# maxrmorrison/torbi

Hardware: AMD Instinct MI355X
Metric: timesteps decoded/sec, 1440 states batch=512 (higher is better)
Workload: dtype f32; 1 GPU; 1440 states, 500 frames, batch=512 per GPU, fp32, dense transition (BASELINE configs[2]); decode = forward + argmax + backtrace, inputs resident in HBM; parallelism=single GPU, streams=2

## Files before the change

torbi_amd/csrc/resident_forward.hpp:

```cpp
#pragma once

#include <hip/hip_runtime.h>
#include <stdint.h>
#include <math.h>
#include <type_traits>

#include "pruned_forward.hpp"
#include "lazy_backtrace.hpp"
#include "nonfinite.hpp"

namespace resident {

using pruned::kBlk;
using pruned::kR;
using pruned::kTop;
using pruned::ListBlock;
using pruned::group_bcast;
using pruned::load_list_block;

constexpr int kNI = 16;
constexpr int kMaxBatches = 16;
constexpr int kRowGroup = 16;
#ifndef TORBI_TILE16_MAX_S
#define TORBI_TILE16_MAX_S pruned::kMaxS16
// ... 100 lines not shown
    if (b >= jb.B) return;
    int f = jb.frames[b];
    f = f < 1 ? 1 : (f > jb.T ? jb.T : f);
    atomicAdd(&jb.hist[f], 1);
}

__global__ __launch_bounds__(1024) void order_large_scan_kernel(OrderJob jb, int ascending) {
    __shared__ int part[1024];
    const int T = jb.T, tid = threadIdx.x;
    const int per = (T + 1024) / 1024;
    auto length_at = [&](int k) { return ascending ? 1 + k : T - k; };
    int sum = 0;
    for (int k = tid * per; k < (tid + 1) * per && k < T; ++k) sum += jb.hist[length_at(k)];
    part[tid] = sum;
    __syncthreads();
    if (tid == 0) {
        int run = 0;
        for (int i = 0; i < 1024; ++i) { const int v = part[i]; part[i] = run; run += v; }
    }
    __syncthreads();
    int run = part[tid];
    for (int k = tid * per; k < (tid + 1) * per && k < T; ++k) {
        const int f = length_at(k), v = jb.hist[f];
        jb.hist[f] = run;
        run += v;
    }
}

__global__ __launch_bounds__(256) void order_large_place_kernel(OrderJob jb) {
    const int b = blockIdx.x * 256 + threadIdx.x;
    if (b >= jb.B) return;
    int f = jb.frames[b];
    f = f < 1 ? 1 : (f > jb.T ? jb.T : f);
    jb.order[atomicAdd(&jb.hist[f], 1)] = b;
}

__global__ __launch_bounds__(256) void order_tiles_kernel(OrderJobs jobs) {
    __shared__ __align__(16) int s_len[kOrderChunk];
    const int w = blockIdx.x * 256 + threadIdx.x;
    if (w < 128) jobs.stats[w] = 0u;
    for (int k = w; k < jobs.nflags; k += gridDim.x * 256) jobs.flags[k] = 0u;
    if ((int)blockIdx.x * 256 >= jobs.tiles) return;
    auto batch_of_tile = [&](int v) {
        int k = 0;
        for (int q = 1; q < jobs.n; ++q)
            if (v >= jobs.job[q].tile0) k = q;
        return k;
    };
    auto tile_length = [&](int k, int j) {
        const OrderJob &jb = jobs.job[k];
        const int last = jobs.ni * j + jobs.ni - 1 < jb.B ? jobs.ni * j + jobs.ni - 1 : jb.B - 1;
        int f = jb.frames[jb.order[jobs.ascending ? last : jobs.ni * j]];
        return f < 1 ? 1 : (f > jb.T ? jb.T : f);
    };
    const bool live = w < jobs.tiles;
    const int k = live ? batch_of_tile(w) : 0;
    const int j = w - jobs.job[k].tile0;
    const int mine = live ? tile_length(k, j) : 1;
    int rank = 0;
    for (int v0 = 0; v0 < jobs.tiles; v0 += kOrderChunk) {
        const int n = min(kOrderChunk, jobs.tiles - v0), n4 = (n + 3) / 4 * 4;
        if (v0) __syncthreads();
        for (int v = threadIdx.x; v < n4; v += 256) {
            const int kv = v < n ? batch_of_tile(v0 + v) : 0;
            s_len[v] = v < n ? tile_length(kv, v0 + v - jobs.job[kv].tile0) : 0;
        }
        __syncthreads();
        for (int v = 0; v < n4; v += 4) {
            const int4 g = *reinterpret_cast<const int4 *>(&s_len[v]);
            rank += (g.x > mine) || (g.x == mine && v0 + v < w);
            rank += (g.y > mine) || (g.y == mine && v0 + v + 1 < w);
            rank += (g.z > mine) || (g.z == mine && v0 + v + 2 < w);
            rank += (g.w > mine) || (g.w == mine && v0 + v + 3 < w);
        }
    }
    if (live) jobs.tile_map[jobs.ascending ? jobs.tiles - 1 - rank : rank] = (k << 20) | j;
}

__global__ __launch_bounds__(256) void absent_kernel(uint4 *__restrict__ slots, size_t granules) {
    const uint4 a = {kAbsentBits, kAbsentBits, kAbsentBits, kAbsentBits};
    for (size_t g = (size_t)blockIdx.x * 256 + threadIdx.x; g < granules; g += (size_t)gridDim.x * 256) slots[g] = a;
}

__device__ __forceinline__ u64 top_key(float v, int state) {
    unsigned u = __float_as_uint(v);
    u ^= (u >> 31) ? 0xffffffffu : 0x80000000u;
    return ((u64)u << 32) | (unsigned)(0x7fffffff - state);
}

template <int KTOP = kTop>
__device__ __forceinline__ void top_insert(u64 *list, u64 x) {
    if (x <= list[KTOP - 1]) return;
#pragma unroll
    for (int r = 0; r < KTOP; ++r) {
        if (x != 0ull) {
            const u64 old = atomicMax(&list[r], x);
            x = old < x ? old : (old == x ? 0ull : x);
        }
    }
}

typedef unsigned int v4u __attribute__((ext_vector_type(4)));
__device__ __forceinline__ void store_through(__amdgpu_buffer_rsrc_t buffer, int offset, float4 v) {
    v4u x = {__float_as_uint(v.x), __float_as_uint(v.y), __float_as_uint(v.z), __float_as_uint(v.w)};
    __builtin_amdgcn_raw_buffer_store_b128(x, buffer, offset, 0, 16);
}
__device__ __forceinline__ void store_plain(__amdgpu_buffer_rsrc_t buffer, int offset, float4 v) {
    v4u x = {__float_as_uint(v.x), __float_as_uint(v.y), __float_as_uint(v.z), __float_as_uint(v.w)};
    __builtin_amdgcn_raw_buffer_store_b128(x, buffer, offset, 0, 0);
}
__device__ __forceinline__ float4 load_through(__amdgpu_buffer_rsrc_t buffer, int offset) {
    const v4u x = __builtin_amdgcn_raw_buffer_load_b128(buffer, offset, 0, 16);
    return make_float4(__uint_as_float(x.x), __uint_as_float(x.y), __uint_as_float(x.z), __uint_as_float(x.w));
}
__device__ __forceinline__ __amdgpu_buffer_rsrc_t buffer_of(const void *base, unsigned bytes) {
    return __builtin_amdgcn_make_buffer_rsrc(const_cast<void *>(base), 0, (int)bytes, 0x00020000);
}

#ifndef RESIDENT_ABL
#define RESIDENT_ABL 0
#endif
#ifndef CLUSTER_POLL_SLEEP
#define CLUSTER_POLL_SLEEP 4
#endif
#ifndef CLUSTER_ROUND
#define CLUSTER_ROUND 8
#endif
#ifndef RESIDENT_EXTRA_VALU
#define RESIDENT_EXTRA_VALU 0
#endif
#ifndef RESIDENT_HORIZON
#define RESIDENT_HORIZON 1
#endif
#ifndef RESIDENT_HORIZON_SLACK
#define RESIDENT_HORIZON_SLACK 2
#endif

#ifndef RESIDENT_PRIO
#define RESIDENT_PRIO 1
#endif
#ifndef RESIDENT_PRIO_CAP
#define RESIDENT_PRIO_CAP 3
#endif
__device__ __forceinline__ int prio_level(int left) {
    const int level = left >= 6 ? 3 : left >= 4 ? 2 : left >= 2 ? 1 : 0;
    return level < RESIDENT_PRIO_CAP ? level : RESIDENT_PRIO_CAP;
}
#ifndef RESIDENT_DEPTH
#define RESIDENT_DEPTH 1
#endif
#ifndef RESIDENT_SPLIT_ADDS
#define RESIDENT_SPLIT_ADDS 0
#endif
constexpr int scan_depth(int MAXP, int KR, bool CLUSTER, int NI) {
    const bool fits = KR == 1 ? !(MAXP == 11 && NI == 8) && !(MAXP == 6 && CLUSTER) : MAXP == 1;
    return RESIDENT_DEPTH >= 2 && fits ? 2 : 1;
}

#ifdef RESIDENT_STAMP
constexpr int kPhases = 12;
__device__ unsigned long long g_phase[1024 * 16 * kPhases];
__device__ unsigned long long g_wgtime[1024 * 4];
#define RSTAMP(i) { const unsigned long long now_ = __builtin_readcyclecounter(); acc[i] += now_ - last; last = now_; }
#define RCOUNT(i, n) acc[i] += (n)
#else
#define RSTAMP(i)
#define RCOUNT(i, n)
#endif

template <int KW, int MAXP, bool PIPE, int KR = kR, bool CLUSTER = false, int NI = 16, bool REPAIR = false>
__global__ __launch_bounds__(64 * KW) void resident_forward_kernel(Group grp, Cluster clu, const float *__restrict__ tt,
                                                                   const float2 *__restrict__ sorted,
                                                                   const float *__restrict__ initial, int S, int SpP) {
    constexpr int kNI = NI, G = NI / 4, EPL = kBlk / G, kRowGroup = 64 / G;
    constexpr int kR = KR, kTop = KR + 1;
    static_assert(NI == 16 || NI == 8, "tiles of 16 or 8 items");
    extern __shared__ __attribute__((aligned(16))) float lds[];
    const int S4 = (S + 3) / 4 * 4;
    u64 *top = reinterpret_cast<u64 *>(lds + (size_t)kNI * S4);
    float *mtopv = reinterpret_cast<float *>(top + kNI * kTop);
    int *mtopi = reinterpret_cast<int *>(mtopv + kNI * kTop);
    int *sframes = mtopi + kNI * kTop;
    int *sitem = sframes + kNI;
    int *smisc = sitem + kNI;

    const int tid = threadIdx.x, lane = tid & 63;
    const int wave = __builtin_amdgcn_readfirstlane(tid >> 6);
    const unsigned long long clock_0 = clock64(), wall_0 = wall_clock64();
#ifdef RESIDENT_STAMP
    const unsigned long long wg_start = wall_clock64();
#endif

    int cid = blockIdx.x, member = 0;
    const int R = CLUSTER ? clu.R : 1;
    if constexpr (REPAIR) {
        if (!grp.only || grp.only[blockIdx.x] == 0u) return;
    }
    bool local = false;
    if constexpr (CLUSTER) {
        const int cls = blockIdx.x & 7;
        if (tid == 0) {
            smisc[0] = (int)__hip_atomic_fetch_add(clu.control + cls, 1u, __ATOMIC_RELAXED, __HIP_MEMORY_SCOPE_AGENT);
            smisc[1] = 0;
        }
        __syncthreads();
        const int ticket = __builtin_amdgcn_readfirstlane(smisc[0]);
        if (clu.spread) {
            const int per = R / 8;
            member = cls * per + ticket % per;
            cid = ticket / per;
        } else {
            member = ticket % R;
            cid = (ticket / R) * 8 + cls;
        }
        if (cid >= clu.tiles) return;
        if (wave == 0) {
            unsigned *const where = clu.where + (size_t)cid * kMaxR;
            const unsigned xcc = __builtin_amdgcn_s_getreg(20 | (0 << 6) | (3 << 11)) & 15u;
            if (lane == 0) __hip_atomic_store(where + member, xcc + 1u, __ATOMIC_RELAXED, __HIP_MEMORY_SCOPE_AGENT);
            unsigned long long since = 0ull;
            unsigned seen = xcc + 1u;
            bool complete = true;
            for (;;) {
                if (lane < R) seen = __hip_atomic_load(where + lane, __ATOMIC_RELAXED, __HIP_MEMORY_SCOPE_AGENT);
                if (__all(seen != 0u)) break;
                const unsigned long long now = wall_clock64();
                if (since == 0ull) since = now;
                if (now - since >= clu.wait_ticks) { complete = false; break; }
                __builtin_amdgcn_s_sleep(8);
            }
            const bool same = complete && __all(seen == xcc + 1u);
            if (lane == 0) smisc[2] = same ? 1 : 0;
        }
        __syncthreads();
#ifndef CLUSTER_LOCAL_EXCHANGE
#define CLUSTER_LOCAL_EXCHANGE 1
#endif
        local = CLUSTER_LOCAL_EXCHANGE && smisc[2] != 0;
    }
    const int code = grp.tile_map[cid];
    const Batch &bat = grp.batch[code >> 20];
    const float *__restrict__ obs = bat.obs;
    float *__restrict__ hist = bat.hist;
    const int B = bat.B, T = bat.T;
    const int b0 = (code & 0xfffff) * kNI;
    bool odd = false;

    if (tid < kNI) {
        int f = 0;
        const int item = bat.order[b0 + tid < B ? b0 + tid : B - 1];
        if (b0 + tid < B) {
            f = bat.frames[item];
            f = f < 1 ? 1 : (f > T ? T : f);
        }
        sframes[tid] = f;
        sitem[tid] = item;
    }
    if (tid < kNI * kTop) top[tid] = 0ull;
    __syncthreads();
    int fmax = 0;
#pragma unroll
    for (int it = 0; it < kNI; ++it) fmax = max(fmax, sframes[it]);

    for (int item = 0; item < kNI; ++item) {
        const int b = sitem[item];
        const bool valid = b0 + item < B;
        const float *src = obs + (size_t)b * T * S;
        float *dst = hist + (size_t)b * T * S;
        for (int i = tid; i < S; i += 64 * KW) {
            const float v = src[i] + initial[i];
            odd = odd || nonfinite::odd(v);
            lds[i * kNI + item] = v;
            if (valid) dst[i] = v;
            top_insert<kTop>(top + item * kTop, top_key(v, i));
        }
    }

    const int g = lane & (G - 1);
    const int jl = G == 4 ? (int)((0xFBAE9DC873261540ull >> (4 * (lane >> 2))) & 15)
                          : (int)((0xFE7654DC32BA9810ull >> (4 * ((lane >> 1) & 15))) & 15) + (lane & 32) / 2;
    const char *ptile = reinterpret_cast<const char *>(lds) + 16 * g;
    const int nrg = (S + kRowGroup - 1) / kRowGroup;
    const int rg_lo = CLUSTER ? cluster_first_group(member, nrg, R) : 0;
    const int rg_hi = CLUSTER ? cluster_first_group(member + 1, nrg, R) : nrg;
    const unsigned xrow = (unsigned)S4 * kNI * (unsigned)sizeof(float);
    const unsigned xbytes = (unsigned)cluster_slot_bytes(S);
    static_assert(kTop <= kMaxTop, "a member publishes at most kMaxTop list entries per item");
    int ib[4];
#pragma unroll
    for (int it = 0; it < 4; ++it) ib[it] = sitem[4 * g + it];

    float pend[MAXP][4];
    const int own_lo = kRowGroup * rg_lo, own_hi = kRowGroup * rg_hi < S ? kRowGroup * rg_hi : S;
    const int pieces = CLUSTER ? (S - (own_hi - own_lo)) * G : 0;
    auto place = [&](int c) {
        int row = c / G;
        row = row < own_lo ? row : row + (own_hi - own_lo);
        return (row * kNI + 4 * (c % G)) * 4;
    };
#ifndef RESIDENT_FIXED8
#define RESIDENT_FIXED8 1
#endif
#ifndef RESIDENT_FIXED16
#define RESIDENT_FIXED16 1
#endif
    constexpr bool FIXED = CLUSTER && MAXP == 1 && (NI == 16 ? RESIDENT_FIXED16 : RESIDENT_FIXED8);
    ListBlock<EPL> head0, head1;
    float obnext[4] = {0.f, 0.f, 0.f, 0.f};
    if constexpr (FIXED) {
        const int rg = rg_lo + wave;
        const int jj = kRowGroup * rg + jl;
        const int jr = (rg < rg_hi && jj < S) ? jj : S - 1;
        const float2 *row = sorted + (size_t)jr * SpP + EPL * g;
        load_list_block(head0, row, 0);
        load_list_block(head1, row, kBlk);
        if (fmax > 1) {
#pragma unroll
            for (int it = 0; it < 4; ++it) obnext[it] = obs[((size_t)ib[it] * T + 1) * S + jr];
        }
    }
    unsigned stat_blocks = 0, stat_passes = 0;
    int horizon[MAXP];
#pragma unroll
    for (int p = 0; p < MAXP; ++p) horizon[p] = 1;

    auto publish_top = [&](int row) {
        if (tid < kNI * kTop) {
            const u64 key = top[tid];
            unsigned u = (unsigned)(key >> 32);
            u ^= (u >> 31) ? 0x80000000u : 0xffffffffu;
            const float value = key ? __uint_as_float(u) : -INFINITY;
            mtopv[tid] = value;
            mtopi[tid] = key ? (0x7fffffff - (int)(unsigned)key) * S : 0;
            top[tid] = 0ull;
            const int item = tid / kTop;
            if (tid == item * kTop && member == 0 && b0 + item < B && row < sframes[item])
                bat.rowmax[(size_t)sitem[item] * T + row] = value;
        }
    };
    __syncthreads();
    publish_top(0);
#ifdef RESIDENT_STAMP
    unsigned long long acc[kPhases] = {};
    unsigned long long last = __builtin_readcyclecounter();
#endif

    constexpr int kPrio = (CLUSTER || REPAIR || MAXP > 8) ? 0 : RESIDENT_PRIO;
    const int npass = __builtin_amdgcn_readfirstlane(wave < nrg ? (nrg - wave + KW - 1) / KW : 0);
    if constexpr (kPrio == 2) {
        if (npass > nrg / KW) __builtin_amdgcn_s_setprio(1);
    }

    for (int t = 1; t < fmax; ++t) {
        __syncthreads();
        RSTAMP(0);

        float seedv[4][kR ? kR : 1], thr[4];
        int seedo[4][kR ? kR : 1];
        bool live[4];
#pragma unroll
        for (int it = 0; it < 4; ++it) {
            const int item = 4 * g + it;
            live[it] = t < sframes[item];
            if constexpr (kTop == 4) {
                const float4 v = *reinterpret_cast<const float4 *>(mtopv + item * kTop);
                const int4 o = *reinterpret_cast<const int4 *>(mtopi + item * kTop);
                const float vv[4] = {v.x, v.y, v.z, v.w};
                const int oo[4] = {o.x, o.y, o.z, o.w};
#pragma unroll
                for (int r = 0; r < kR; ++r) { seedv[it][r] = vv[r]; seedo[it][r] = oo[r]; }
                thr[it] = live[it] ? vv[kR] : -INFINITY;
            } else {
#pragma unroll
                for (int r = 0; r < kR; ++r) { seedv[it][r] = mtopv[item * kTop + r]; seedo[it][r] = mtopi[item * kTop + r]; }
                thr[it] = live[it] ? mtopv[item * kTop + kR] : -INFINITY;
            }
        }
        RSTAMP(1);

        int opaque = 0;
        asm volatile("" : "+s"(opaque));
#pragma unroll
        for (int p = 0; p < MAXP; ++p) {
            const int rg = rg_lo + wave + KW * p + opaque;
            if (rg < rg_hi) {
                if constexpr (kPrio == 1) {
                    const int left = npass - p;
                    const int level = prio_level(left);
                    if (p == 0 || level != prio_level(left + 1)) {
                        if (level == 3) __builtin_amdgcn_s_setprio(3);
                        else if (level == 2) __builtin_amdgcn_s_setprio(2);
                        else if (level == 1) __builtin_amdgcn_s_setprio(1);
                        else if (p != 0) __builtin_amdgcn_s_setprio(0);
                    }
                }
                const int jj = kRowGroup * rg + jl;
                const bool jv = jj < S;
                const int jr = jv ? jj : S - 1;
                const float2 *row = sorted + (size_t)jr * SpP + EPL * g;
                ListBlock<EPL> cur, nxt;
                float ob[4];
                if constexpr (FIXED) {
                    cur = head0;
                    nxt = head1;
#pragma unroll
                    for (int it = 0; it < 4; ++it) ob[it] = obnext[it];
                } else {
                    load_list_block(cur, row, 0);
                    load_list_block(nxt, row, kBlk);
#pragma unroll
                    for (int it = 0; it < 4; ++it)
                        ob[it] = (RESIDENT_ABL & 32) ? 0.5f * it : obs[((size_t)ib[it] * T + t) * S + jr];
                }
                float seedt[4][kR ? kR : 1];
#pragma unroll
                for (int it = 0; it < 4; ++it)
#pragma unroll
                    for (int r = 0; r < kR; ++r)
                        seedt[it][r] = (RESIDENT_ABL & 64) ? -1.0f : tt[(unsigned)(seedo[it][r] + jr)];

                float best[4] = {-INFINITY, -INFINITY, -INFINITY, -INFINITY};
#if RESIDENT_EXTRA_VALU
                float dummy[4] = {0.f, 0.f, 0.f, 0.f};
#endif
                struct PairData { float4 p0, p1; float t0, t1; };
                auto issue = [&](auto Hc, const ListBlock<EPL> &blk, PairData &d) {
                    constexpr int H = decltype(Hc)::value, O = H / (EPL / 2), E = H % (EPL / 2);
                    float t0, t1;
                    int o0, o1;
                    if (RESIDENT_ABL & 4) {
                        t0 = blk.e[E].x; t1 = blk.e[E].z; o0 = __float_as_int(blk.e[E].y); o1 = __float_as_int(blk.e[E].w);
                    } else {
                        t0 = group_bcast<G, O>(blk.e[E].x); t1 = group_bcast<G, O>(blk.e[E].z);
                        o0 = group_bcast<G, O>(__float_as_int(blk.e[E].y));
                        o1 = group_bcast<G, O>(__float_as_int(blk.e[E].w));
                    }
                    asm volatile("" : "+v"(t0), "+v"(t1));
                    d.t0 = t0; d.t1 = t1;
                    if (RESIDENT_ABL & 2) {
                        d.p0 = make_float4(__int_as_float(o0), t1, t0, t1);
                        d.p1 = make_float4(__int_as_float(o1), t0, t1, t0);
                    } else {
                        d.p0 = *reinterpret_cast<const float4 *>(ptile + o0);
                        d.p1 = *reinterpret_cast<const float4 *>(ptile + o1);
                    }
                };
                auto math = [&](const PairData &d) {
#if RESIDENT_EXTRA_VALU
#pragma unroll
                    for (int x = 0; x < RESIDENT_EXTRA_VALU; ++x) asm volatile("v_add_f32 %0, %0, %1" : "+v"(dummy[x & 3]) : "v"(d.t0));
#endif
                    if (RESIDENT_SPLIT_ADDS) {
                        float a0 = d.t0 + d.p0.x, a1 = d.t0 + d.p0.y, a2 = d.t0 + d.p0.z, a3 = d.t0 + d.p0.w;
                        float b0 = d.t1 + d.p1.x, b1 = d.t1 + d.p1.y, b2 = d.t1 + d.p1.z, b3 = d.t1 + d.p1.w;
                        asm volatile("" : "+v"(a0), "+v"(a1), "+v"(a2), "+v"(a3), "+v"(b0), "+v"(b1), "+v"(b2), "+v"(b3));
                        best[0] = fmaxf(fmaxf(best[0], a0), b0);
                        best[1] = fmaxf(fmaxf(best[1], a1), b1);
                        best[2] = fmaxf(fmaxf(best[2], a2), b2);
                        best[3] = fmaxf(fmaxf(best[3], a3), b3);
                        return;
                    }
                    best[0] = fmaxf(fmaxf(best[0], d.t0 + d.p0.x), d.t1 + d.p1.x);
                    best[1] = fmaxf(fmaxf(best[1], d.t0 + d.p0.y), d.t1 + d.p1.y);
                    best[2] = fmaxf(fmaxf(best[2], d.t0 + d.p0.z), d.t1 + d.p1.z);
                    best[3] = fmaxf(fmaxf(best[3], d.t0 + d.p0.w), d.t1 + d.p1.w);
                };
                PairData ahead;
                PairData ahead1;
                constexpr int kDepth = PIPE ? scan_depth(MAXP, KR, CLUSTER, NI) : 1;
                auto consume = [&](const ListBlock<EPL> &blk, const ListBlock<EPL> &after) {
                    if constexpr (kDepth == 2) {
                        PairData fresh;
#define TORBI_STAGE(H_, BLK_)                                                                  \
                        issue(std::integral_constant<int, (H_ + 2) % 8>(), BLK_, fresh);       \
                        __builtin_amdgcn_sched_barrier(0);                                     \
                        math(ahead);                                                           \
                        __builtin_amdgcn_sched_barrier(0);                                     \
                        ahead = ahead1;                                                        \
                        ahead1 = fresh;
                        TORBI_STAGE(0, blk)
                        TORBI_STAGE(1, blk)
                        TORBI_STAGE(2, blk)
                        TORBI_STAGE(3, blk)
                        TORBI_STAGE(4, blk)
                        TORBI_STAGE(5, blk)
                        TORBI_STAGE(6, after)
                        TORBI_STAGE(7, after)
#undef TORBI_STAGE
                    } else if (PIPE) {
                        PairData other;
#define TORBI_STAGE(H_, CUR_, NXT_)                                                   \
                        issue(std::integral_constant<int, H_ + 1>(), blk, NXT_);      \
                        __builtin_amdgcn_sched_barrier(0);                            \
                        math(CUR_);                                                   \
                        __builtin_amdgcn_sched_barrier(0);
                        TORBI_STAGE(0, ahead, other)
                        TORBI_STAGE(1, other, ahead)
                        TORBI_STAGE(2, ahead, other)
                        TORBI_STAGE(3, other, ahead)
                        TORBI_STAGE(4, ahead, other)
                        TORBI_STAGE(5, other, ahead)
                        TORBI_STAGE(6, ahead, other)
#undef TORBI_STAGE
                        issue(std::integral_constant<int, 0>(), after, ahead);
                        __builtin_amdgcn_sched_barrier(0);
                        math(other);
                        __builtin_amdgcn_sched_barrier(0);
                    } else {
                        PairData d;
                        issue(std::integral_constant<int, 0>(), blk, d); math(d);
                        issue(std::integral_constant<int, 1>(), blk, d); math(d);
                        issue(std::integral_constant<int, 2>(), blk, d); math(d);
                        issue(std::integral_constant<int, 3>(), blk, d); math(d);
                        issue(std::integral_constant<int, 4>(), blk, d); math(d);
                        issue(std::integral_constant<int, 5>(), blk, d); math(d);
                        issue(std::integral_constant<int, 6>(), blk, d); math(d);
                        issue(std::integral_constant<int, 7>(), blk, d); math(d);
                    }
                };
                if (PIPE) issue(std::integral_constant<int, 0>(), cur, ahead);
                if constexpr (kDepth == 2) issue(std::integral_constant<int, 1>(), cur, ahead1);
                int nblk = 1;
                consume(cur, nxt);
                load_list_block(cur, row, 2 * kBlk);
                auto fold_seeds = [&]() {
#pragma unroll
                    for (int it = 0; it < 4; ++it)
#pragma unroll
                        for (int r = 0; r < kR; ++r) best[it] = fmaxf(best[it], seedv[it][r] + seedt[it][r]);
                };
                const int first_test = RESIDENT_HORIZON ? horizon[p] : 1;
                auto more = [&](const ListBlock<EPL> &blk) {
                    if (RESIDENT_ABL & 1) return nblk < 11;
                    if (RESIDENT_HORIZON && nblk < first_test) return true;
                    const float tn = group_bcast<G, 0>(blk.e[0].x);
                    return (bool)__any(jv && ((tn + thr[0] > best[0]) | (tn + thr[1] > best[1]) | (tn + thr[2] > best[2]) |
                                              (tn + thr[3] > best[3])));
                };
                const int Sp = (S + 15) / 16 * 16;
                fold_seeds();
                RSTAMP(2);
                for (int kk = kBlk; kk < Sp; kk += 2 * kBlk) {
                    if (!more(nxt)) break;
                    RCOUNT(7, 1);
                    ++nblk;
                    consume(nxt, cur);
                    load_list_block(nxt, row, kk + 2 * kBlk);
                    if (!more(cur)) break;
                    RCOUNT(7, 1);
                    ++nblk;
                    consume(cur, nxt);
                    load_list_block(cur, row, kk + 3 * kBlk);
                }
                if ((t & 15) == 1) { stat_blocks += (unsigned)nblk; stat_passes += 1u; }
                if (RESIDENT_HORIZON)
                    horizon[p] = __builtin_amdgcn_readfirstlane(max(1, nblk - RESIDENT_HORIZON_SLACK));
                RSTAMP(3);
                u64 last4[4];
#pragma unroll
                for (int it = 0; it < 4; ++it) last4[it] = top[(4 * g + it) * kTop + kTop - 1];
#pragma unroll
                for (int it = 0; it < 4; ++it) {
#if RESIDENT_EXTRA_VALU
                    if (dummy[it] == 12345.678f) best[it] = 0.f;
#endif
                    const float o = ob[it] + best[it];
                    odd = odd || nonfinite::odd(o);
                    pend[p][it] = o;
                    if (jv && live[it] && !(RESIDENT_ABL & 8)) hist[((size_t)ib[it] * T + t) * S + jr] = o;
                    const u64 key = top_key(o, jr);
                    if (jv && key > last4[it] && !(RESIDENT_ABL & 16)) top_insert<kTop>(top + (4 * g + it) * kTop, key);
                }
                RSTAMP(4);
            }
        }
        if constexpr (CLUSTER) {
            if (t + 1 < fmax && !(RESIDENT_ABL & 128)) {
                const __amdgpu_buffer_rsrc_t xdst = buffer_of(
                    reinterpret_cast<const char *>(clu.xchg) + (size_t)(kSlots * cid + (t & (kSlots - 1))) * xbytes, xrow);
#pragma unroll
                for (int p = 0; p < MAXP; ++p) {
                    const int rg = rg_lo + wave + KW * p + opaque;
                    const int jj = kRowGroup * rg + jl;
                    if (rg < rg_hi && jj < S) {
                        const float4 row4 = make_float4(pend[p][0], pend[p][1], pend[p][2], pend[p][3]);
                        if (local) store_plain(xdst, (jj * kNI + 4 * g) * 4, row4);
                        else store_through(xdst, (jj * kNI + 4 * g) * 4, row4);
                    }
                }
            }
            RSTAMP(8);
        }
        __syncthreads();
        RSTAMP(5);
#pragma unroll
        for (int p = 0; p < MAXP; ++p) {
            const int rg = rg_lo + wave + KW * p + opaque;
            const int jj = kRowGroup * rg + jl;
            if (rg < rg_hi && jj < S)
                *reinterpret_cast<float4 *>(lds + (size_t)jj * kNI + 4 * g) =
                    make_float4(pend[p][0], pend[p][1], pend[p][2], pend[p][3]);
        }
        if constexpr (CLUSTER) {
            if (t + 1 < fmax) {
                const __amdgpu_buffer_rsrc_t xold = buffer_of(
                    reinterpret_cast<const char *>(clu.xchg) + (size_t)(kSlots * cid + ((t + 2) & (kSlots - 1))) * xbytes, xrow);
                unsigned absent_bits = kAbsentBits;
                asm volatile("" : "+v"(absent_bits));
                const float absent = __uint_as_float(absent_bits);
                const float4 none = make_float4(absent, absent, absent, absent);
#pragma unroll
                for (int p = 0; p < MAXP; ++p) {
                    const int rg = rg_lo + wave + KW * p + opaque;
                    const int jj = kRowGroup * rg + jl;
                    if (rg < rg_hi && jj < S) {
                        if (local) store_plain(xold, (jj * kNI + 4 * g) * 4, none);
                        else store_through(xold, (jj * kNI + 4 * g) * 4, none);
                    }
                }
                asm volatile("" ::: "memory");
            }
        }
        if constexpr (FIXED) {
            if (t + 1 < fmax) {
                const int jj = kRowGroup * (rg_lo + wave) + jl;
                const int jr = (rg_lo + wave < rg_hi && jj < S) ? jj : S - 1;
#pragma unroll
                for (int it = 0; it < 4; ++it) obnext[it] = obs[((size_t)ib[it] * T + t + 1) * S + jr];
            }
        }
        if constexpr (CLUSTER) {
            if (t + 1 < fmax) {
                const __amdgpu_buffer_rsrc_t xsrc = buffer_of(
                    reinterpret_cast<const char *>(clu.xchg) + (size_t)(kSlots * cid + (t & (kSlots - 1))) * xbytes, xbytes);
                if (wave == 0 && lane < kNI * kTop) {
                    const u64 k = top[lane];
                    v4u x = {(unsigned)k, (unsigned)t, (unsigned)(k >> 32), (unsigned)t};
                    const int at = (int)xrow + (member * kNI * kMaxTop + lane) * 16;
                    if (local) __builtin_amdgcn_raw_buffer_store_b128(x, xsrc, at, 0, 0);
                    else __builtin_amdgcn_raw_buffer_store_b128(x, xsrc, at, 0, 16);
                }
                RSTAMP(6);
                {
                    const int kpair = kNI * kTop / 2;
                    const int km = tid / kpair, ks = tid - km * kpair;
                    bool want_keys = km < R && km != member;
                    const bool keyed = want_keys;
                    v4u key0 = {0u, 0u, 0u, 0u}, key1 = {0u, 0u, 0u, 0u};
                    const int kat = (int)xrow + (km * kNI * kMaxTop + 2 * ks) * 16;
                    constexpr int kRound = CLUSTER_ROUND;
                    unsigned spins = 0;
                    unsigned long long since = 0ull;
                    bool gave_up = false;
                    for (int first = 0; first < pieces && !gave_up; first += kRound * 64 * KW) {
                        float4 got[kRound];
                        unsigned missing = 0u;
#pragma unroll
                        for (int u = 0; u < kRound; ++u) {
                            missing |= (first + tid + u * 64 * KW < pieces ? 1u : 0u) << u;
                            got[u] = make_float4(0.f, 0.f, 0.f, 0.f);
                        }
                        for (;;) {
#pragma unroll
                            for (int u = 0; u < kRound; ++u)
                                if (missing >> u & 1u) got[u] = load_through(xsrc, place(first + tid + u * 64 * KW));
                            if (want_keys) {
                                key0 = __builtin_amdgcn_raw_buffer_load_b128(xsrc, kat, 0, 16);
                                key1 = __builtin_amdgcn_raw_buffer_load_b128(xsrc, kat + 16, 0, 16);
                            }
#pragma unroll
                            for (int u = 0; u < kRound; ++u) {
                                const bool there = __float_as_uint(got[u].x) != kAbsentBits && __float_as_uint(got[u].y) != kAbsentBits &&
                                                   __float_as_uint(got[u].z) != kAbsentBits && __float_as_uint(got[u].w) != kAbsentBits;
                                if (there) missing &= ~(1u << u);
                            }
                            if (want_keys && key0.y == (unsigned)t && key0.w == (unsigned)t && key1.y == (unsigned)t &&
                                key1.w == (unsigned)t)
                                want_keys = false;
                            if (!__any(missing != 0u || want_keys)) break;
                            RCOUNT(9, 1);
                            __builtin_amdgcn_s_sleep(CLUSTER_POLL_SLEEP);
                            if ((spins++ & 15u) == 0u) {
                                const unsigned long long now = wall_clock64();
                                if (since == 0ull) since = now;
                                if (now - since >= clu.wait_ticks) {
                                    if (lane == 0) smisc[1] = 1;
                                    gave_up = true;
                                    break;
                                }
                            }
                        }
#pragma unroll
                        for (int u = 0; u < kRound; ++u) {
                            const int c = first + tid + u * 64 * KW;
                            if (c < pieces) *reinterpret_cast<float4 *>(reinterpret_cast<char *>(lds) + place(c)) = got[u];
                        }
                    }
                    if (keyed && !gave_up) {
                        const u64 k0 = ((u64)key0.z << 32) | key0.x, k1 = ((u64)key1.z << 32) | key1.x;
                        if (k0) top_insert<kTop>(top + (2 * ks / kTop) * kTop, k0);
                        if (k1) top_insert<kTop>(top + ((2 * ks + 1) / kTop) * kTop, k1);
                    }
                }
                RSTAMP(10);
                __syncthreads();
                RSTAMP(11);
                if (smisc[1]) break;
            }
        }
        publish_top(t);
        RSTAMP(6);
    }
    if constexpr (kPrio == 2) __builtin_amdgcn_s_setprio(0);
    if constexpr (CLUSTER) {
        if (tid == 0 && smisc[1]) {
            atomicAdd(&grp.stats[127], 1u);
            clu.failed[cid] = 1u;
        }
    }
    if (lane == 0 && stat_passes) {
        atomicAdd(&grp.stats[0], stat_blocks);
        atomicAdd(&grp.stats[64], stat_passes);
// ... 66 lines not shown
```

torbi_amd/csrc/torbi_hip.hip:

```cpp

#include <hip/hip_runtime.h>
#include <algorithm>
#include <atomic>
#include <mutex>
#include <type_traits>
#include <vector>
#include <stdint.h>
#include <stddef.h>
#include <math.h>
#include <stdlib.h>

#include "torbi_hip.h"
#include "scratch.hpp"
#include "dispatch.hpp"
#include "dense_forward.hpp"
#include "lazy_backtrace.hpp"
#include "uniform_decode.hpp"
#include "pruned_forward.hpp"
#include "resident_forward.hpp"
#include "small_batch_forward.hpp"
#include "held_matrix_forward.hpp"
#include "small_states.hpp"
#include "band_forward.hpp"
#include "band_tile_forward.hpp"
// ... 824 lines not shown
        return by_flag(env ? atoi(env) != 0 : B > cus * (NB * PQ >= 9 ? 1 : 8), [&](auto pairs) {
            constexpr int NSEQ = decltype(pairs)::value ? 2 : 1;
            auto *kernel = &small::block_value_kernel<PQ, L, NSEQ>;
            TORBI_NOTE_KERNEL("small::block_value_kernel<%d, %d, %d>", PQ, L, NSEQ);
            hipLaunchKernelGGL(kernel, dim3((B + NSEQ - 1) / NSEQ), dim3(64 * NB * PQ), 0, stream, obs, frames, trans, init,
                               reinterpret_cast<float *>(w.trellis), w.post[0], w.post[1], record, (int)ROUTE_SMALL, B, T, S, NB,
                               t_serial);
            return hipGetLastError();
        });
    }); });
    if (e != hipSuccess) return e;
    const float *hist = reinterpret_cast<const float *>(w.trellis);
    const bool vec = (S % 4 == 0) && ((reinterpret_cast<uintptr_t>(trans) & 15) == 0);
    const int K = (vec && w.arrive) ? std::min(backtrace_segments(B), 8) : 1;
    if (K > 1) {
        hipLaunchKernelGGL(lazy::segment_rows_kernel<1>, dim3(B * K), dim3(64), 0, stream, hist, trans, frames, out, B, T, S, K,
                           w.arrive);
        hipLaunchKernelGGL(lazy::stitch_rows_kernel<1>, dim3(B), dim3(64), 0, stream, hist, trans, frames, out, B, T, S, K, w.arrive);
        return hipGetLastError();
    }
    return launch_backtrace_on(hist, trans, frames, out, B, T, S, stream, nullptr, nullptr);
}

template <int BL, int JL, int NW, int KC, int MSL>
hipError_t launch_dense_steps(const float *obs, const int32_t *frames, const DenseWorkspace &w,
                              int B, int T, int S, hipStream_t stream, int *launches, unsigned *clock_out) {
    const dense::Plan &pl = w.plan;
    const size_t lds = dense::lds_bytes<BL, JL, NW, KC, MSL>();
    auto *kernel = &dense::step_dense_kernel<BL, JL, NW, KC, MSL>;
    hipError_t e = ensure_dynamic_lds(kernel, lds);
    if (e != hipSuccess) return e;
    TORBI_NOTE_KERNEL("dense::step_dense_kernel<%d, %d, %d, %d, %d>", BL, JL, NW, KC, MSL);
    const int ntiles = pl.n_bt * pl.n_jt;
    const int grid = 8 * ((ntiles + 7) / 8);
    int n = 0;
    for (int t = 1; t < T; ++t) {
        hipLaunchKernelGGL(kernel, dim3(grid), dim3(64 * NW), lds, stream, obs, frames, w.trp, w.panel[(t - 1) & 1],
                           w.panel[t & 1], w.hist, w.chunks, B, T, S, t, pl.n_bt, pl.n_jt, pl.JT, pl.Kp, pl.NCH, pl.RB, clock_out);
        ++n;
    }
    if (launches) *launches = n;
    return hipGetLastError();
}

hipError_t launch_dense_forward(const float *obs, const int32_t *frames, const float *trans,
                                const float *init, const DenseWorkspace &w, int B, int T, int S,
                                hipStream_t stream, int *launches, bool reuse, unsigned *clock_out) {
    const dense::Plan &pl = w.plan;
    if (!reuse) {
        hipLaunchKernelGGL(dense::pack_transition_kernel, dim3((pl.Kp + 63) / 64, pl.n_jt), dim3(256), 0,
                           stream, trans, w.trp, S, pl.JT, pl.W, pl.Kp);
        hipLaunchKernelGGL(dense::build_chunk_lists_kernel, dim3(pl.n_jt), dim3(256),
                           sizeof(int) * (size_t)pl.NCH, stream, w.trp, w.chunks, S, pl.JT, pl.W, pl.Kp, pl.NCH,
                           pl.KC);
        hipLaunchKernelGGL(stamp_route_kernel, dim3(1), dim3(1), 0, stream, w.widest, 0);
        hipLaunchKernelGGL(lazy::row_ranges_kernel, dim3(S), dim3(64), 0, stream, trans, w.ranges, w.widest, S);
    }
    {
        const size_t n = (size_t)pl.n_bt * pl.BT * pl.Kp;
        const int grid = (int)((n + 255) / 256 < 4096 ? (n + 255) / 256 : 4096);
        hipLaunchKernelGGL(dense::init_panels_kernel, dim3(grid), dim3(256), 0, stream, obs, init,
                           w.panel[0], w.panel[1], w.hist, B, T, S, pl.n_bt, pl.BT, pl.Kp);
    }
    hipError_t e = hipGetLastError();
    if (e != hipSuccess) return e;
    return by_value<6, 4, 2>(pl.JL, [&](auto jl) {
        constexpr int BL = 8, JL = decltype(jl)::value, NW = 8, KC = 12, MSL = 8;
        if (pl.BL != BL || pl.JL != JL || pl.NW != NW || pl.KC != KC || pl.MSL != MSL) return hipErrorInvalidValue;
        return launch_dense_steps<BL, JL, NW, KC, MSL>(obs, frames, w, B, T, S, stream, launches, clock_out);
    });
}

void launch_list_preparation(const float *trans, float2 *sorted, int32_t *row_range, float *tt, int S, int SpP, int NPOW,
                             int items_per_tile, hipStream_t stream) {
    hipLaunchKernelGGL(pruned::sort_rows_kernel, dim3(S), dim3(256), sizeof(float) * 2 * (size_t)NPOW, stream, trans,
                       sorted, row_range, S, SpP, NPOW, items_per_tile * 4);
    if (items_per_tile == pruned::kNB) {
        const int n = (S / 4) * (SpP / pruned::kBlk);
        hipLaunchKernelGGL(pruned::arrange_blocks_kernel<4>, dim3((n + 63) / 64), dim3(64), 0, stream, sorted, S, SpP);
    } else {
        const int n = (S / 8) * (SpP / pruned::kBlk);
        hipLaunchKernelGGL(pruned::arrange_blocks_kernel<8>, dim3((n + 63) / 64), dim3(64), 0, stream, sorted, S, SpP);
    }
    hipLaunchKernelGGL(pruned::transpose_kernel, dim3((S + 31) / 32, (S + 31) / 32), dim3(256), 0, stream, trans, tt, S);
}

hipError_t launch_backtrace_on(const float *hist, const float *trans, const int32_t *frames, int32_t *out,
                               int B, int T, int S, hipStream_t stream, const int32_t *ranges = nullptr,
                               const int32_t *widest = nullptr) {
    const bool vec = (S % 4 == 0) && ((reinterpret_cast<uintptr_t>(trans) & 15) == 0);
    if (vec && S <= 256 * 16) {
        if (!ranges) widest = nullptr;
        by_state_count<2, 6, 16>(S, [&](auto nq) {
            constexpr int NQ = decltype(nq)::value;
            if (ranges)
                hipLaunchKernelGGL(lazy::backtrace_ranged_kernel<NQ>, dim3(B), dim3(64), 0, stream, hist, trans, ranges,
                                   widest, frames, out, B, T, S);
            hipLaunchKernelGGL(lazy::backtrace_prefetch_kernel<NQ>, dim3(B), dim3(64), 0, stream, hist,
                               trans, frames, out, B, T, S, widest);
        });
        return hipGetLastError();
    }
    if (vec)
        hipLaunchKernelGGL(lazy::backtrace_kernel<4>, dim3(B), dim3(64), 0, stream, hist, trans,
                           frames, out, B, T, S);
    else
        hipLaunchKernelGGL(lazy::backtrace_kernel<1>, dim3(B), dim3(64), 0, stream, hist, trans,
                           frames, out, B, T, S);
    return hipGetLastError();
}

hipError_t launch_backtrace_sorted(const float *hist, const float2 *sorted, int SpP, int items_per_tile,
                                   const float *trans, const int32_t *frames, int32_t *out, int B, int T, int S,
                                   hipStream_t stream, const float *rowmax) {
    if (S % 4 != 0 || S > 256 * 16)
        return launch_backtrace_on(hist, trans, frames, out, B, T, S, stream);
    const int shift = items_per_tile == pruned::kNB ? 6 : 5;
    by_state_count(S, [&](auto nq) {
        hipLaunchKernelGGL(lazy::backtrace_gather_kernel<decltype(nq)::value>, dim3(B), dim3(64), 0, stream, hist, rowmax, sorted,
                           SpP, shift, frames, out, B, T, S);
    });
    return hipGetLastError();
}

struct HostBatch {
    const float *obs;
    const int32_t *frames;
    int32_t *out;
    void *workspace;
    int B, T;
    int32_t *record;
};

inline bool few_seeds(unsigned flags, bool clusters) {
    if (flags & TORBI_HIP_FEW_SEEDS) return true;
    if (flags & TORBI_HIP_MANY_SEEDS) return false;
    return clusters;
}

template <int KW, int MAXP, int KR, bool CLUSTER, int NI, bool REPAIR = false>
hipError_t launch_resident_kernel(const resident::Group &grp, const resident::Cluster &clu, int workgroups,
                                  const ResidentWorkspace &w, const float *init, int S, hipStream_t stream) {
    const size_t lds = resident::lds_bytes(S, KR + 1);
    auto *kernel = &resident::resident_forward_kernel<KW, MAXP, true, KR, CLUSTER, NI, REPAIR>;
    const hipError_t e = ensure_dynamic_lds(kernel, lds);
    if (e != hipSuccess) return e;
    hipLaunchKernelGGL(kernel, dim3(workgroups), dim3(64 * KW), lds, stream, grp, clu, w.tt, w.sorted, init, S, w.SpP);
    if (!REPAIR)
        TORBI_NOTE_KERNEL("resident::resident_forward_kernel<%d, %d, true, %d, %s, %d, false>", KW, MAXP, KR,
                          CLUSTER ? "true" : "false", NI);
    return hipGetLastError();
}

template <int KR, int NI>
hipError_t launch_whole_tiles(const resident::Group &grp, const resident::Cluster &clu, int tiles, const ResidentWorkspace &w,
                              const float *init, int S, hipStream_t s) {
    const int nrg = (S + resident::pass_rows(S) - 1) / resident::pass_rows(S);
    if constexpr (NI != resident::kNI) {
        if (nrg <= 96) return launch_resident_kernel<12, 8, KR, false, NI>(grp, clu, tiles, w, init, S, s);
        return launch_resident_kernel<12, 11, KR, false, NI>(grp, clu, tiles, w, init, S, s);
    } else {
        if (nrg <= 72) return launch_resident_kernel<12, 6, KR, false, NI>(grp, clu, tiles, w, init, S, s);
        if (nrg <= 96) return launch_resident_kernel<12, 8, KR, false, NI>(grp, clu, tiles, w, init, S, s);
        return launch_resident_kernel<12, 11, KR, false, NI>(grp, clu, tiles, w, init, S, s);
    }
}

inline int backtrace_segments(int items) {
    const char *e = getenv("TORBI_HIP_BACKTRACE_SEGMENTS");
    const int wanted = e ? atoi(e) : 8;
    if (wanted <= 1 || items > 1024) return 1;
    return std::max(2, std::min(wanted, 2048 / std::max(items, 1)));
}

inline hipError_t nonfinite_begin(const HostBatch *hb, int n, const float *trans, const float *init, int S, hipStream_t s,
                                  bool scan_observations, int reach_left = -1, int reach_right = -1, bool scan_matrix = true,
                                  float background = -INFINITY) {
    const int serial = new_serial();
    if (!scan_matrix) return hipSuccess;
    nonfinite::Records recs{};
    recs.n = n;
    for (int k = 0; k < n; ++k) recs.record[k] = hb[k].record;
    const size_t cells = (size_t)S * S;
    hipLaunchKernelGGL(nonfinite::matrix_kernel, dim3((unsigned)std::max<size_t>(1, std::min<size_t>(1024, (cells + 2047) / 2048))),
                       dim3(256), 0, s, trans, init, S, recs, serial, reach_left, reach_right, background);
    if (scan_observations)
        for (int k = 0; k < n; ++k) {
            const size_t count = (size_t)hb[k].B * hb[k].T * S;
            hipLaunchKernelGGL(nonfinite::observation_kernel,
                               dim3((unsigned)std::max<size_t>(1, std::min<size_t>(2048, (count + 4095) / 4096))), dim3(256), 0, s,
                               hb[k].obs, count, recs.record[k], serial);
        }
    return hipGetLastError();
}
inline hipError_t nonfinite_end(const HostBatch *hb, int n, const float *trans, const float *init, int S, hipStream_t s) {
    nonfinite::RepairJobs jobs{};
    jobs.n = n;
    int items = 0;
    for (int k = 0; k < n; ++k) {
        jobs.obs[k] = hb[k].obs;
        jobs.frames[k] = hb[k].frames;
        jobs.out[k] = hb[k].out;
        jobs.trellis[k] = static_cast<int32_t *>(hb[k].workspace);
        jobs.record[k] = hb[k].record;
        jobs.rows[k] = reinterpret_cast<float *>(reinterpret_cast<char *>(jobs.record[k]) + 256);
        jobs.B[k] = hb[k].B;
        jobs.T[k] = hb[k].T;
        jobs.item0[k] = items;
        items += hb[k].B;
    }
    hipLaunchKernelGGL(nonfinite::repair_kernel, dim3(items), dim3(256), 0, s, jobs, trans, init, S, t_serial);
    return hipGetLastError();
}

inline unsigned long long cluster_wait_ticks() {
    const char *e = getenv("TORBI_HIP_CLUSTER_WAIT_US");
    return e ? 100ull * strtoull(e, nullptr, 10) : resident::kClusterWaitTicks;
}

struct LaunchGroup {
    resident::Group grp;
    int tiles, items;
};
hipError_t assemble_group(const HostBatch *hb, int n, int S, int cus, hipStream_t s, bool ascending, int items_per_tile,
                          Route route, unsigned *flags, int nflags, LaunchGroup &g) {
    resident::Group &grp = g.grp;
    resident::OrderJobs jobs{};
    grp = resident::Group{};
    grp.n = n;
    grp.serial = t_serial;
    int tiles = 0, items = 0, widest = 0;
    for (int k = 0; k < n; ++k) {
        resident::Batch &b = grp.batch[k];
        const ResidentWorkspace wk = carve_resident(hb[k].workspace, hb[k].B, hb[k].T, S, cus);
        b.alarm = hb[k].record + nonfinite::kAlarmWord;
        b.obs = hb[k].obs;
        b.frames = hb[k].frames;
        b.out = hb[k].out;
        b.hist = wk.hist;
        b.order = wk.order;
        b.rowmax = wk.rowmax;
        jobs.job[k] = resident::OrderJob{hb[k].frames, wk.order, hb[k].B, hb[k].T, tiles, wk.lengths_hist, hb[k].record, (int)route};
        widest = std::max(widest, hb[k].B);
        b.B = hb[k].B;
        b.T = hb[k].T;
        b.tile0 = tiles;
        b.item0 = items;
        tiles += (hb[k].B + items_per_tile - 1) / items_per_tile;
        items += hb[k].B;
    }
    if (tiles > kMaxGroupTiles) return hipErrorInvalidValue;
    g.tiles = tiles;
    g.items = items;
    const ResidentWorkspace w = carve_resident(hb[0].workspace, hb[0].B, hb[0].T, S, cus);
    grp.tile_map = w.tile_map;
    grp.stats = w.stats;
    jobs.ascending = ascending ? 1 : 0;
    jobs.stats = w.stats;
    jobs.n = n;
    jobs.tiles = tiles;
    jobs.tile_map = w.tile_map;
    jobs.ni = items_per_tile;
    jobs.flags = flags;
    jobs.nflags = nflags;
    hipLaunchKernelGGL(resident::order_items_kernel, dim3((widest + 255) / 256, n), dim3(256), 0, s, jobs);
    for (int k = 0; k < n; ++k) {
        const resident::OrderJob &jb = jobs.job[k];
        if (jb.B <= resident::kMaxOrdered) continue;
        const ResidentWorkspace wk = carve_resident(hb[k].workspace, hb[k].B, hb[k].T, S, cus);
        hipError_t me = hipMemsetAsync(wk.lengths_hist, 0, wk.lengths_hist_bytes, s);
        if (me != hipSuccess) return me;
        hipLaunchKernelGGL(resident::order_large_count_kernel, dim3((jb.B + 255) / 256), dim3(256), 0, s, jb);
        hipLaunchKernelGGL(resident::order_large_scan_kernel, dim3(1), dim3(1024), 0, s, jb, jobs.ascending);
        hipLaunchKernelGGL(resident::order_large_place_kernel, dim3((jb.B + 255) / 256), dim3(256), 0, s, jb);
    }
    hipLaunchKernelGGL(resident::order_tiles_kernel, dim3((tiles + 255) / 256), dim3(256), 0, s, jobs);
    return hipSuccess;
}

hipError_t run_resident(const HostBatch *hb, int n, const float *trans, const float *init, int S, int cus, hipStream_t s,
                        hipEvent_t *ev, int *launches, bool reuse, bool ascending, bool clusters, bool few,
                        Preparation *kept) {
    {
        const hipError_t ne = nonfinite_begin(hb, n, trans, init, S, s, false);
        if (ne != hipSuccess) return ne;
    }
    int tiles = 0;
    for (int k = 0; k < n; ++k) tiles += tiles_of(hb[k].B, S);
    const ResidentWorkspace w = carve_resident(hb[0].workspace, hb[0].B, hb[0].T, S, cus, kept);
    const int R = clusters ? cluster_members(tiles, S, cus) : 1;
    const int spread = (R % 8 == 0 && resident::tile_items(S) == 8) ? 1 : 0;
    resident::Cluster clu{w.xchg, w.where, tiles, w.control, w.failed, R, cluster_wait_ticks(), spread};
    if (ev) (void)hipEventRecord(ev[0], s);
    if (kept) reuse = kept->valid;
    if (!reuse) launch_list_preparation(trans, w.sorted, w.row_range, w.tt, S, w.SpP, w.NPOW, resident::tile_items(S), s);
    if (kept) kept->valid = true;
    LaunchGroup group;
    hipError_t e = assemble_group(hb, n, S, cus, s, ascending, resident::tile_items(S), R > 1 ? ROUTE_CLUSTER : ROUTE_RESIDENT,
                                  w.flags, R > 1 ? w.nflags : 0, group);
    if (e != hipSuccess) return e;
    const resident::Group &grp = group.grp;
    const int items = group.items;
    if (ev) (void)hipEventRecord(ev[3], s);
    const int nrg = (S + resident::pass_rows(S) - 1) / resident::pass_rows(S);
    const bool small = resident::tile_items(S) != resident::kNI;
    e = by_flag(few, [&](auto few_) { return by_flag(small, [&](auto small_) {
        constexpr int KR = decltype(few_)::value ? 1 : 3, NI = decltype(small_)::value ? 8 : resident::kNI;
        if (R <= 1) return launch_whole_tiles<KR, NI>(grp, clu, tiles, w, init, S, s);
        {
            const size_t granules = (size_t)tiles * resident::kSlots * resident::cluster_slot_bytes(S) / 16;
            hipLaunchKernelGGL(resident::absent_kernel, dim3((unsigned)std::min<size_t>((granules + 255) / 256, 2048)), dim3(256),
                               0, s, reinterpret_cast<uint4 *>(w.xchg), granules);
        }
        const int passes = ((nrg + R - 1) / R + 11) / 12;
        const int grid = 8 * ((tiles + 7) / 8) * R;
        const int share = (nrg + R - 1) / R;
        hipError_t ce;
        if constexpr (NI == 8) {
            if (share <= 8) ce = launch_resident_kernel<8, 1, KR, true, NI>(grp, clu, grid, w, init, S, s);
            else if (share <= 16) ce = launch_resident_kernel<8, 2, KR, true, NI>(grp, clu, grid, w, init, S, s);
            else if (passes <= 2) ce = launch_resident_kernel<12, 2, KR, true, NI>(grp, clu, grid, w, init, S, s);
            else if (passes <= 4) ce = launch_resident_kernel<12, 4, KR, true, NI>(grp, clu, grid, w, init, S, s);
            else ce = launch_resident_kernel<12, 6, KR, true, NI>(grp, clu, grid, w, init, S, s);
        } else if (passes <= 1) ce = launch_resident_kernel<12, 1, KR, true, NI>(grp, clu, grid, w, init, S, s);
        else if (passes <= 2) ce = launch_resident_kernel<12, 2, KR, true, NI>(grp, clu, grid, w, init, S, s);
        else if (passes <= 4) ce = launch_resident_kernel<12, 4, KR, true, NI>(grp, clu, grid, w, init, S, s);
        else ce = launch_resident_kernel<12, 6, KR, true, NI>(grp, clu, grid, w, init, S, s);
        if (ce != hipSuccess) return ce;
        resident::Group again = grp;
        again.only = clu.failed;
        return launch_resident_kernel<12, 11, KR, false, NI, true>(again, clu, tiles, w, init, S, s);
    }); });
    if (launches) *launches = 1;
    if (ev) (void)hipEventRecord(ev[1], s);
    if (e != hipSuccess) return e;
    const int K = backtrace_segments(items);
    if (S % 4 == 0 && K > 1) {
        int32_t *const arrive = w.tile_map;
        by_state_count(S, [&](auto nq) {
            constexpr int NQ = decltype(nq)::value;
            hipLaunchKernelGGL(resident::group_segment_gather_kernel<NQ>, dim3(items * K), dim3(64), 0, s, grp, w.sorted, w.SpP, S, K,
                               arrive);
            hipLaunchKernelGGL(resident::group_stitch_gather_kernel<NQ>, dim3(items), dim3(64), 0, s, grp, w.sorted, w.SpP, S, K, arrive);
        });
    } else if (S % 4 == 0) {
        by_state_count(S, [&](auto nq) {
            hipLaunchKernelGGL(resident::group_backtrace_gather_kernel<decltype(nq)::value>, dim3(items), dim3(64), 0, s, grp, w.sorted,
                               w.SpP, S);
        });
    } else
        hipLaunchKernelGGL(resident::group_backtrace_kernel<1>, dim3(items), dim3(64), 0, s, grp, trans, S);
    {
        const hipError_t ne = nonfinite_end(hb, n, trans, init, S, s);
        if (ne != hipSuccess) return ne;
    }
    if (ev) (void)hipEventRecord(ev[2], s);
    return hipGetLastError();
}


inline int band_tiles(int B) { return (B + band::kNI - 1) / band::kNI; }

struct BandChoice {
    band::Plan pl;
    band::TilePlan tile;
    bool whole;
    int cap;
    float background;
};
inline bool choose_band(int S, int hl, int hr, int tiles, int cus, BandChoice &c, float background = -INFINITY) {
    c = BandChoice{};
    c.background = background;
    if (tiles < 1 || background != background || background == INFINITY) return false;
    const char *force = getenv("TORBI_HIP_BAND_FORM");
    const char *tw = getenv("TORBI_HIP_TILE_WAVES");
    const bool tile_ok = band::make_tile_plan(S, hl, hr, c.tile, tw ? atoi(tw) : 0) && !(force && force[0] == 's');
    band::Plan split{};
    const bool split_ok = !(force && force[0] == 't' && tile_ok) && band::make_plan(S, hl, hr, tiles, cus, split, background) &&
                          band::tiles_per_launch(split, cus) >= 1;
    const int per = split_ok ? std::max(1, std::min(band::tiles_per_launch(split, cus), kMaxGroupTiles)) : 1;
    const bool enough = split_ok ? 8 * ((tiles + per - 1) / per) >= 5 * split.R : 2 * tiles >= cus;
    if (tile_ok && (enough || (force && force[0] == 't'))) {
        c.whole = true;
        c.pl.S = S; c.pl.hl = hl; c.pl.hr = hr; c.pl.R = 1;
        c.cap = tiles;
        c.tile.background = background;
        return true;
    }
    if (!split_ok) return false;
    c.pl = split;
    c.cap = std::min(band::tiles_per_launch(c.pl, cus), kMaxGroupTiles);
    return true;
}

hipError_t run_band(const HostBatch *hb, int n, const float *trans, const float *init, int S, const BandChoice &choice, int cus,
                    hipStream_t s, hipEvent_t *ev, int *launches, bool ascending) {
    const band::Plan &pl = choice.pl;
    band::Exchange ex{};
    band::ClearJobs clear{};
    {
        const hipError_t ne = nonfinite_begin(hb, n, trans, init, S, s, false, pl.hl, pl.hr, true, choice.background);
        if (ne != hipSuccess) return ne;
    }
    size_t most = 0;
    for (int k = 0; k < n; ++k) {
        const BandWorkspace wk = carve_band(hb[k].workspace, hb[k].B, hb[k].T, S, cus);
        ex.xchg[k] = wk.xchg;
        clear.xchg[k] = wk.xchg;
        clear.bytes[k] = pl.R > 1 && !choice.whole ? band::xchg_bytes(hb[k].B, S) : 0;
        most = std::max(most, clear.bytes[k]);
    }
    const BandWorkspace w = carve_band(hb[0].workspace, hb[0].B, hb[0].T, S, cus);
    if (ev) (void)hipEventRecord(ev[0], s);
    LaunchGroup group;
    hipError_t e = assemble_group(hb, n, S, cus, s, ascending, band::kNI, ROUTE_BAND, nullptr, 0, group);
    if (e != hipSuccess) return e;
    const resident::Group &grp = group.grp;
    const int tiles = group.tiles, items = group.items;
    const int nlaunch = choice.whole ? 1 : (tiles + choice.cap - 1) / choice.cap;
    ex.failed = w.failed;
    ex.wait_ticks = cluster_wait_ticks();
    clear.words = w.words;
    clear.nwords = 16 + kMaxGroupTiles + 8 * nlaunch;
    clear.n = n;
    if (choice.whole) {
        const band::TilePlan &tp = choice.tile;
        hipLaunchKernelGGL(band::pack_band_kernel, dim3(tp.nblk * tp.Dq4), dim3(64), 0, s, trans, w.tpack, S, tp.hl, tp.hr, tp.Dq,
                           tp.Dq4);
        if (ev) (void)hipEventRecord(ev[3], s);
        e = by_value<1, 2, 3>(tp.bpw, [&](auto bpw) { return by_flag(tp.waves == 12, [&](auto twelve) {
            return by_flag(tp.background != -INFINITY, [&](auto bg) {
                constexpr int BPW = decltype(bpw)::value, NW = BPW == 1 || (BPW == 2 && decltype(twelve)::value) ? 12 : 8;
                constexpr bool BG = decltype(bg)::value;
                auto *kernel = &band::band_tile_kernel<BPW, NW, BG>;
                const hipError_t le = ensure_dynamic_lds(kernel, (size_t)tp.lds_bytes);
                if (le != hipSuccess) return le;
                TORBI_NOTE_KERNEL("band::band_tile_kernel<%d, %d, %s>", BPW, NW, BG ? "true" : "false");
                hipLaunchKernelGGL(kernel, dim3(tiles), dim3(64 * tp.waves), (size_t)tp.lds_bytes, s, grp, tp, w.tpack, init);
                return hipSuccess;
            });
        }); });
        if (e != hipSuccess) return e;
    } else {
        {
            const size_t blocks = std::max<size_t>(1, std::min<size_t>(2048, (most / 16 + 255) / 256));
            hipLaunchKernelGGL(band::clear_exchange_kernel, dim3((unsigned)blocks, n), dim3(256), 0, s, clear);
        }
        if (ev) (void)hipEventRecord(ev[3], s);
        e = by_flag(choice.background != -INFINITY, [&](auto bg) {
            constexpr bool BG = decltype(bg)::value;
            auto *kernel = &band::band_forward_kernel<BG>;
            const hipError_t le = ensure_dynamic_lds(kernel, (size_t)pl.lds_bytes);
            if (le != hipSuccess) return le;
            TORBI_NOTE_KERNEL("band::band_forward_kernel<%s>", BG ? "true" : "false");
            for (int l = 0; l < nlaunch; ++l) {
                ex.tile0 = l * choice.cap;
                ex.tiles = std::min(tiles, ex.tile0 + choice.cap);
                ex.control = w.tickets + 8 * l;
                const int here = ex.tiles - ex.tile0;
                const int grid = pl.R > 1 ? 8 * ((here + 7) / 8) * pl.R : here;
                hipLaunchKernelGGL(kernel, dim3(grid), dim3(64 * pl.waves), (size_t)pl.lds_bytes, s, grp, ex, pl, trans, init);
// ... 1050 lines not shown
```

Before: 60.83 million timesteps/s.

## Use 16-wave resident kernel for mid-size state counts and reload item indices

```diff
diff --git a/torbi_amd/csrc/resident_forward.hpp b/torbi_amd/csrc/resident_forward.hpp
--- a/torbi_amd/csrc/resident_forward.hpp
+++ b/torbi_amd/csrc/resident_forward.hpp
@@ -276,6 +276,9 @@
 #ifndef RESIDENT_SPLIT_ADDS
 #define RESIDENT_SPLIT_ADDS 0
 #endif
+#ifndef RESIDENT_RELOAD_ITEMS
+#define RESIDENT_RELOAD_ITEMS 1
+#endif
 constexpr int scan_depth(int MAXP, int KR, bool CLUSTER, int NI) {
     const bool fits = KR == 1 ? !(MAXP == 11 && NI == 8) && !(MAXP == 6 && CLUSTER) : MAXP == 1;
     return RESIDENT_DEPTH >= 2 && fits ? 2 : 1;
@@ -410,9 +413,21 @@
     const unsigned xrow = (unsigned)S4 * kNI * (unsigned)sizeof(float);
     const unsigned xbytes = (unsigned)cluster_slot_bytes(S);
     static_assert(kTop <= kMaxTop, "a member publishes at most kMaxTop list entries per item");
+    constexpr bool kReloadItems = RESIDENT_RELOAD_ITEMS && KW > 12 && !CLUSTER;
     int ib[4];
 #pragma unroll
     for (int it = 0; it < 4; ++it) ib[it] = sitem[4 * g + it];
+    auto items_now = [&](int (&now)[4]) {
+        if constexpr (kReloadItems) {
+            int at = 4 * g;
+            asm volatile("" : "+v"(at));
+            const int4 v = *reinterpret_cast<const int4 *>(sitem + at);
+            now[0] = v.x; now[1] = v.y; now[2] = v.z; now[3] = v.w;
+        } else {
+#pragma unroll
+            for (int it = 0; it < 4; ++it) now[it] = ib[it];
+        }
+    };
 
     float pend[MAXP][4];
     const int own_lo = kRowGroup * rg_lo, own_hi = kRowGroup * rg_hi < S ? kRowGroup * rg_hi : S;
@@ -532,9 +547,11 @@
                 } else {
                     load_list_block(cur, row, 0);
                     load_list_block(nxt, row, kBlk);
+                    int in[4];
+                    items_now(in);
 #pragma unroll
                     for (int it = 0; it < 4; ++it)
-                        ob[it] = (RESIDENT_ABL & 32) ? 0.5f * it : obs[((size_t)ib[it] * T + t) * S + jr];
+                        ob[it] = (RESIDENT_ABL & 32) ? 0.5f * it : obs[((size_t)in[it] * T + t) * S + jr];
                 }
                 float seedt[4][kR ? kR : 1];
 #pragma unroll
@@ -683,6 +700,8 @@
                 u64 last4[4];
 #pragma unroll
                 for (int it = 0; it < 4; ++it) last4[it] = top[(4 * g + it) * kTop + kTop - 1];
+                int out[4];
+                items_now(out);
 #pragma unroll
                 for (int it = 0; it < 4; ++it) {
 #if RESIDENT_EXTRA_VALU
@@ -691,7 +710,7 @@
                     const float o = ob[it] + best[it];
                     odd = odd || nonfinite::odd(o);
                     pend[p][it] = o;
-                    if (jv && live[it] && !(RESIDENT_ABL & 8)) hist[((size_t)ib[it] * T + t) * S + jr] = o;
+                    if (jv && live[it] && !(RESIDENT_ABL & 8)) hist[((size_t)out[it] * T + t) * S + jr] = o;
                     const u64 key = top_key(o, jr);
                     if (jv && key > last4[it] && !(RESIDENT_ABL & 16)) top_insert<kTop>(top + (4 * g + it) * kTop, key);
                 }
diff --git a/torbi_amd/csrc/torbi_hip.hip b/torbi_amd/csrc/torbi_hip.hip
--- a/torbi_amd/csrc/torbi_hip.hip
+++ b/torbi_amd/csrc/torbi_hip.hip
@@ -1000,15 +1000,34 @@
     return hipGetLastError();
 }
 
+#ifndef TORBI_WHOLE_TILE_WAVES
+#define TORBI_WHOLE_TILE_WAVES 16
+#endif
+inline int whole_tile_waves(int nrg, int tiles, int cus) {
+    if (nrg <= 72 || nrg > 96) return 12;
+    int waves = 2 * tiles > cus ? TORBI_WHOLE_TILE_WAVES : 12;
+    if (const char *e = getenv("TORBI_HIP_WHOLE_TILE_WAVES")) {
+        const int asked = atoi(e);
+        if (asked == 12 || asked == 15 || asked == 16) waves = asked;
+    }
+    if (waves == 15 && nrg > 90) waves = 12;
+    return waves;
+}
+
 template <int KR, int NI>
 hipError_t launch_whole_tiles(const resident::Group &grp, const resident::Cluster &clu, int tiles, const ResidentWorkspace &w,
-                              const float *init, int S, hipStream_t s) {
+                              const float *init, int S, int cus, hipStream_t s) {
     const int nrg = (S + resident::pass_rows(S) - 1) / resident::pass_rows(S);
     if constexpr (NI != resident::kNI) {
         if (nrg <= 96) return launch_resident_kernel<12, 8, KR, false, NI>(grp, clu, tiles, w, init, S, s);
         return launch_resident_kernel<12, 11, KR, false, NI>(grp, clu, tiles, w, init, S, s);
     } else {
         if (nrg <= 72) return launch_resident_kernel<12, 6, KR, false, NI>(grp, clu, tiles, w, init, S, s);
+        if constexpr (KR == 1) {
+            const int waves = whole_tile_waves(nrg, tiles, cus);
+            if (waves == 16) return launch_resident_kernel<16, 6, KR, false, NI>(grp, clu, tiles, w, init, S, s);
+            if (waves == 15) return launch_resident_kernel<15, 6, KR, false, NI>(grp, clu, tiles, w, init, S, s);
+        }
         if (nrg <= 96) return launch_resident_kernel<12, 8, KR, false, NI>(grp, clu, tiles, w, init, S, s);
         return launch_resident_kernel<12, 11, KR, false, NI>(grp, clu, tiles, w, init, S, s);
     }
@@ -1154,7 +1173,7 @@
     const bool small = resident::tile_items(S) != resident::kNI;
     e = by_flag(few, [&](auto few_) { return by_flag(small, [&](auto small_) {
         constexpr int KR = decltype(few_)::value ? 1 : 3, NI = decltype(small_)::value ? 8 : resident::kNI;
-        if (R <= 1) return launch_whole_tiles<KR, NI>(grp, clu, tiles, w, init, S, s);
+        if (R <= 1) return launch_whole_tiles<KR, NI>(grp, clu, tiles, w, init, S, cus, s);
         {
             const size_t granules = (size_t)tiles * resident::kSlots * resident::cluster_slot_bytes(S) / 16;
             hipLaunchKernelGGL(resident::absent_kernel, dim3((unsigned)std::min<size_t>((granules + 255) / 256, 2048)), dim3(256),
```

Result: faster. 62.03 million timesteps/s (median of 6 runs) (+2.0%).
